# naver/dust3r

Measured on NVIDIA H100. Metric: image-pairs/sec (512x384, ViT-L/B+DPT), higher is better.
Workload: dtype bf16

## Files before the change

dust3r_b200/_lib.py:

```python
from __future__ import annotations

import ctypes as C
import os

from ._lib_fwd import Model

_HERE = os.path.dirname(os.path.abspath(__file__))
LIB_PATH = os.path.join(_HERE, 'libdust3r_b200.so')

_lib = None


class D3RError(RuntimeError):
    pass


class AlignDesc(C.Structure):
    _fields_ = [
        ('n_imgs', C.c_int32), ('n_edges', C.c_int32), ('n_entries', C.c_int32), ('n_chunks', C.c_int32),
        ('max_deg', C.c_int32), ('max_chunks', C.c_int32), ('chunk_px', C.c_int32), ('dist_l2', C.c_int32), ('norm_pw_scale', C.c_int32),
        ('tied_focal', C.c_int32), ('eval_only', C.c_int32),
        ('base_scale', C.c_float), ('pw_break', C.c_float), ('focal_break', C.c_float), ('adam_eps', C.c_float),
        ('beta1', C.c_float), ('beta2', C.c_float),
        ('img_hw', C.c_void_p), ('img_pix_off', C.c_void_p), ('img_ent_ptr', C.c_void_p),
# ... 52 lines not shown
    'd3r_align_stream_warps_per_cta': (i32, []),
    'd3r_align_stream_max_window': (i32, []),
    'd3r_align_pack_entries': (i32, [vp, i32, i32, i32, i32, vp, vp]),
    'd3r_gemm_bf16': (i32, [vp, vp, vp, vp, vp, vp, i32, i32, i32, i64, u32, vp, vp, i32, i32, i32, vp]),
    'd3r_conv3x3_bf16': (i32, [vp, vp, vp, vp, vp, vp, vp, i32, i32, i32, i32, i32, u32, vp]),
    'd3r_attention_hd64': (i32, [vp, i64, vp, i64, vp, i64, vp, i64, i32, i32, i32, i32, f32, vp]),
    'd3r_conv_transpose_bf16': (i32, [vp, vp, vp, vp, i32, i32, i32, i32, i32, i32, vp]),
    'd3r_conv3x3_head_tail': (i32, [vp, vp, vp, vp, vp, vp, vp, i32, i32, i32, i32, i32, f32, f32, vp]),
    'd3r_layernorm_bf16': (i32, [vp, vp, vp, vp, i32, i32, f32, vp]),
    'd3r_upsample2x_bf16': (i32, [vp, vp, i32, i32, i32, i32, i32, i32, vp]),
    'd3r_im2col_3x3_s2_bf16': (i32, [vp, vp, i32, i32, i32, i32, vp]),
    'd3r_patch_im2col16': (i32, [vp, vp, i32, i32, i32, vp]),
    'd3r_linear_head_postprocess': (i32, [vp, vp, vp, i32, i32, i32, i32, i32, i32, f32, f32, vp]),
    'd3r_set_gemm_impl': (None, [i32]),
    'd3r_set_gemm_store': (None, [i32]),
    'd3r_set_conv_store': (None, [i32]),
    'd3r_set_attention_impl': (None, [i32]),
    'd3r_clean_pointcloud': (i32, [i32, vp, vp, i32, vp, vp, vp, vp, vp, f32, f32, vp]),
    'd3r_procrustes_moments': (i32, [i32, i32, vp, vp, vp, vp, vp]),
    'd3r_weiszfeld_focal': (i32, [i32, i32, i32, vp, vp, i32, vp, vp]),
    'd3r_nearest_neighbours': (i32, [i32, i32, vp, vp, vp, vp]),
    'd3r_image_resize_crop_normalize': (i32, [vp, i32, i32, i32, i32, vp, vp, i32, vp, vp, i32, i32, i32, i32, i32, i32, i32,
                                              vp, vp, vp, vp]),
    'd3r_sizeof_jpeg_desc': (i32, []),
    'd3r_jpeg_decode_workspace_bytes': (i64, [_JPEG, i64]),
    'd3r_jpeg_decode': (i32, [_JPEG, vp, i64, vp, vp, vp, i64, vp]),
    'd3r_segment_sky_workspace_bytes': (i64, [i32, i64]),
    'd3r_segment_sky': (i32, [i32, vp, vp, i32, i64, vp, vp, vp, i64, vp]),
    'd3r_nanmedian_workspace_bytes': (i64, [i32]),
    'd3r_segmented_nanmedian': (i32, [i32, i64, vp, vp, vp, i64, vp]),
# ... 88 lines not shown
```

dust3r_b200/csrc/gemm_host.cu:

```cuda
#include "gemm_wgmma.cuh"
#include "gemm_host.h"
#include "prof.h"

namespace d3r {
namespace gemm {

static int pick_block_n(int N, int mode, uint32_t flags, int conv_m_tiles = 0) {
  if (flags & F_HEAD_FINAL) return 128;
  if (conv_m_tiles > 0) return (N == 256 && (conv_m_tiles + 1) / 2 >= 4 * (num_sms() / 2)) ? 256 : 128;
  if (N % 256 == 0 && pick_epi(mode, flags) != EPI_GENERIC) return 256;
  if (N % 128 == 0) return 128;
  if (N % 64 == 0) return 64;
  return (N > 128) ? 128 : 64;
}

static int g_impl = 2;
constexpr int kPairMinKb = 4;
static bool use_pair(int bn, int num_kb) { return bn >= 128 && (g_impl == 1 || (g_impl == 2 && num_kb >= kPairMinKb)); }

static int g_store = 1;
static int g_conv_store = 1;

static int grid_for(bool pair, int m_tiles, int n_tiles) {
  if (pair) {
    const int items = ((m_tiles + 1) / 2) * n_tiles;
    const int max_clusters = num_sms() / 2;
    return 2 * (items < max_clusters ? items : max_clusters);
  }
  const int items = m_tiles * n_tiles;
  return items < num_sms() ? items : num_sms();
}

static const char* prof_tag(const Params& p, int bn, bool pair) {
  return (p.mode == 1) ? ((p.flags & F_HEAD_FINAL) ? (pair ? "conv3x3_head_tail_2cta" : "conv3x3_head_tail")
                                                   : (pair ? "conv3x3_wgmma_2cta" : "conv3x3_wgmma"))
                       : (bn == 256 ? (pair ? "gemm_wgmma_2cta_bn256" : "gemm_wgmma_bn256")
                                    : (pair ? "gemm_wgmma_2cta_bn128" : (bn == 128 ? "gemm_wgmma_bn128" : "gemm_wgmma_bn64")));
}

template <int BN, int EPI, bool PAIR, bool TMA_STORE = false>
static int launch(const CUtensorMap& ta, const CUtensorMap& tb, const CUtensorMap& to, const Params& p, int m_tiles, int n_tiles,
                  cudaStream_t st) {
  constexpr int kSmem = Cfg<BN, TMA_STORE>::kSmemBytes;
  static unsigned long long attr_devices = 0;
  if (first_launch_on_this_device(attr_devices))
    D3R_CUDA(cudaFuncSetAttribute(gemm_kernel<BN, EPI, PAIR, TMA_STORE>, cudaFuncAttributeMaxDynamicSharedMemorySize, kSmem));
  const int grid = grid_for(PAIR, m_tiles, n_tiles);
  char detail[96];
  snprintf(detail, sizeof(detail), "M=%d N=%d K=%d flags=0x%x mode=%d epi=%d", p.M, p.N, p.K, (unsigned)p.flags, p.mode, EPI);
  prof::Scope scope(prof_tag(p, BN, PAIR), st, 2.0 * double(p.M) * double(p.N) * double(p.K), 0.0, 1, detail);
  D3R_CUDA(pdl::launch_clustered(gemm_kernel<BN, EPI, PAIR, TMA_STORE>, dim3(grid), dim3(kNumThreads), size_t(kSmem), st, PAIR ? 2 : 1,
                                 ta, tb, to, p));
  D3R_LAUNCH_CHECK();
  return D3R_OK;
}

template <int BN, bool PAIR>
static int launch_conv(const CUtensorMap& ta, const CUtensorMap& tb, const CUtensorMap& to, const ConvMaps& cm, const Params& p,
                       int m_tiles, int n_tiles, cudaStream_t st) {
  constexpr int kSmem = Cfg<BN, true>::kSmemBytes;
  static unsigned long long attr_devices = 0;
  if (first_launch_on_this_device(attr_devices))
    D3R_CUDA(cudaFuncSetAttribute(conv_kernel<BN, PAIR>, cudaFuncAttributeMaxDynamicSharedMemorySize, kSmem));
  const int grid = grid_for(PAIR, m_tiles, n_tiles);
  char detail[96];
  snprintf(detail, sizeof(detail), "M=%d N=%d K=%d flags=0x%x mode=%d epi=%d", p.M, p.N, p.K, (unsigned)p.flags, p.mode, EPI_GENERIC);
  prof::Scope scope(prof_tag(p, BN, PAIR), st, 2.0 * double(p.M) * double(p.N) * double(p.K), 0.0, 1, detail);
  D3R_CUDA(pdl::launch_clustered(conv_kernel<BN, PAIR>, dim3(grid), dim3(kNumThreads), size_t(kSmem), st, PAIR ? 2 : 1, ta, tb, to, cm, p));
  D3R_LAUNCH_CHECK();
  return D3R_OK;
}

template <int BN, bool PAIR>
static int dispatch_epi(int epi, const CUtensorMap& ta, const CUtensorMap& tb, const CUtensorMap* to, const Params& p, int m_tiles,
                        int n_tiles, cudaStream_t st) {
  if constexpr (BN == 256) {
    if (to) {
      switch (epi) {
        case EPI_RESID: return launch<BN, EPI_RESID, PAIR, true>(ta, tb, *to, p, m_tiles, n_tiles, st);
        case EPI_ACT: return launch<BN, EPI_ACT, PAIR, true>(ta, tb, *to, p, m_tiles, n_tiles, st);
        case EPI_ROPE: return launch<BN, EPI_ROPE, PAIR, true>(ta, tb, *to, p, m_tiles, n_tiles, st);
      }
    }
  }
  switch (epi) {
    case EPI_RESID: return launch<BN, EPI_RESID, PAIR>(ta, tb, tb, p, m_tiles, n_tiles, st);
    case EPI_ACT: return launch<BN, EPI_ACT, PAIR>(ta, tb, tb, p, m_tiles, n_tiles, st);
    case EPI_ROPE: return launch<BN, EPI_ROPE, PAIR>(ta, tb, tb, p, m_tiles, n_tiles, st);
  }
  if constexpr (BN == 128) return launch<128, EPI_GENERIC, PAIR>(ta, tb, tb, p, m_tiles, n_tiles, st);
  set_error("no BLOCK_N %d kernel for the generic epilogue", BN);
  return D3R_ERR_INVALID;
}

static int dispatch(int bn, const CUtensorMap& ta, const CUtensorMap& tb, const CUtensorMap* to, const Params& p, int m_tiles,
                    cudaStream_t st) {
  const int n_tiles = (p.N + bn - 1) / bn;
  const int epi = (bn >= 128) ? pick_epi(p.mode, p.flags) : EPI_GENERIC;
  const bool pair = use_pair(bn, p.num_kb);
  switch (bn) {
    case 256: return pair ? dispatch_epi<256, true>(epi, ta, tb, to, p, m_tiles, n_tiles, st) : dispatch_epi<256, false>(epi, ta, tb, to, p, m_tiles, n_tiles, st);
    case 128: return pair ? dispatch_epi<128, true>(epi, ta, tb, nullptr, p, m_tiles, n_tiles, st) : dispatch_epi<128, false>(epi, ta, tb, nullptr, p, m_tiles, n_tiles, st);
    case 64: return launch<64, EPI_GENERIC, false>(ta, tb, tb, p, m_tiles, n_tiles, st);
  }
  set_error("unsupported BLOCK_N %d", bn);
  return D3R_ERR_INVALID;
}

static int make_tmap_b(CUtensorMap* m, const void* B, int N, int taps, int Kc, int bn, int num_kb, const char* op) {
  cuuint64_t dims[3] = {(cuuint64_t)Kc, (cuuint64_t)taps, (cuuint64_t)N};
  cuuint64_t str[2] = {(cuuint64_t)Kc * 2, (cuuint64_t)taps * Kc * 2};
  cuuint32_t box[3] = {(cuuint32_t)BLOCK_K, 1, (cuuint32_t)(use_pair(bn, num_kb) ? bn / 2 : bn)};
  return encode_tensor_map(m, B, 3, dims, str, box, op);
}

int gemm_bf16(const void* A, long long lda, const void* B, Params p, cudaStream_t st) {
  D3R_CHECK_ARG(A && B, "gemm: null operand");
  D3R_CHECK_ARG(p.M > 0 && p.N > 0 && p.K > 0, "gemm: bad shape %d %d %d", p.M, p.N, p.K);
  D3R_CHECK_ARG(p.N % 32 == 0, "gemm: N=%d must be a multiple of 32", p.N);
  D3R_CHECK_ARG(p.K % 8 == 0 && lda % 8 == 0, "gemm: K=%d / lda=%lld must be multiples of 8 (16-byte TMA strides)", p.K, lda);
  D3R_CHECK_ARG((reinterpret_cast<uintptr_t>(A) & 15) == 0 && (reinterpret_cast<uintptr_t>(B) & 15) == 0, "gemm: operands must be 16-byte aligned");
  p.mode = 0;
  p.num_kb = (p.K + BLOCK_K - 1) / BLOCK_K;
  const int bn = pick_block_n(p.N, p.mode, p.flags);
  CUtensorMap ta, tb;
  {
    cuuint64_t dims[2] = {(cuuint64_t)p.K, (cuuint64_t)p.M};
    cuuint64_t str[1] = {(cuuint64_t)lda * 2};
    cuuint32_t box[2] = {(cuuint32_t)BLOCK_K, (cuuint32_t)BLOCK_M};
    int rc = encode_tensor_map(&ta, A, 2, dims, str, box, "gemm");
    if (rc) return rc;
  }
  int rc = make_tmap_b(&tb, B, p.N, 1, p.K, bn, p.num_kb, "gemm");
  if (rc) return rc;
  CUtensorMap to;
  const bool f32 = (p.flags & F_RESID_INPLACE) != 0;
  const long long row_bytes = p.ldo * (f32 ? 4 : 2);
  const bool staged = g_store == 1 && bn == 256 && pick_epi(p.mode, p.flags) != EPI_GENERIC && p.ldo >= p.N && row_bytes % 16 == 0 &&
                      (reinterpret_cast<uintptr_t>(p.out) & 15) == 0;
  if (staged) {
    cuuint64_t dims[2] = {(cuuint64_t)p.N, (cuuint64_t)p.M};
    cuuint64_t str[1] = {(cuuint64_t)row_bytes};
    cuuint32_t box[2] = {(cuuint32_t)(f32 ? 32 : 64), 64};
    rc = encode_tensor_map(&to, p.out, 2, dims, str, box, "gemm output", f32 ? CU_TENSOR_MAP_DATA_TYPE_FLOAT32 : CU_TENSOR_MAP_DATA_TYPE_BFLOAT16);
    if (rc) return rc;
  }
  return dispatch(bn, ta, tb, staged ? &to : nullptr, p, (p.M + BLOCK_M - 1) / BLOCK_M, st);
}

static int make_tmap_conv_io(CUtensorMap* m, const void* base, int B, int H, int W, int C, int tile_w, const char* op) {
  const int bw = tile_w < 64 ? tile_w : 64;
  cuuint64_t dims[4] = {(cuuint64_t)C, (cuuint64_t)W, (cuuint64_t)H, (cuuint64_t)B};
  cuuint64_t str[3] = {(cuuint64_t)C * 2, (cuuint64_t)W * C * 2, (cuuint64_t)H * W * C * 2};
  cuuint32_t box[4] = {64, (cuuint32_t)bw, (cuuint32_t)(64 / bw), 1};
  return encode_tensor_map(m, base, 4, dims, str, box, op);
}

static bool aligned16(const void* ptr) { return (reinterpret_cast<uintptr_t>(ptr) & 15) == 0; }

int conv3x3_bf16(const void* x_nhwc, const void* w_packed, int B, int H, int W, int Cin, int Cout, Params p, cudaStream_t st) {
  D3R_CHECK_ARG(x_nhwc && w_packed, "conv3x3: null operand");
  D3R_CHECK_ARG(Cin % 8 == 0 && Cout % 32 == 0, "conv3x3: Cin=%d must be a multiple of 8 and Cout=%d of 32", Cin, Cout);
// ... 12 lines not shown
  p.tiles_y = (H + p.tile_h - 1) / p.tile_h;
  p.ldo = Cout;
  const int m_tiles = B * p.tiles_x * p.tiles_y;
  const bool staged = g_conv_store == 1 && (Cout == 256 || Cout == 128) && (p.flags & ~EpiMask<EPI_CONV>::value) == 0 &&
                      aligned16(p.out) && (!(p.flags & F_OUT2_RELU) || aligned16(p.out2)) && (!(p.flags & F_ADD0) || aligned16(p.add0)) &&
                      (!(p.flags & F_ADD1) || aligned16(p.add1));
  const int bn = pick_block_n(p.N, p.mode, p.flags, staged ? m_tiles : 0);
  CUtensorMap ta, tb;
  {
    cuuint64_t dims[4] = {(cuuint64_t)Cin, (cuuint64_t)W, (cuuint64_t)H, (cuuint64_t)B};
    cuuint64_t str[3] = {(cuuint64_t)Cin * 2, (cuuint64_t)W * Cin * 2, (cuuint64_t)H * W * Cin * 2};
    cuuint32_t box[4] = {(cuuint32_t)BLOCK_K, (cuuint32_t)p.tile_w, (cuuint32_t)p.tile_h, 1};
    int rc = encode_tensor_map(&ta, x_nhwc, 4, dims, str, box, "conv3x3");
    if (rc) return rc;
  }
  int rc = make_tmap_b(&tb, w_packed, Cout, 9, Cin, bn, p.num_kb, "conv3x3");
  if (rc) return rc;
  if (!staged) return dispatch(bn, ta, tb, nullptr, p, m_tiles, st);
  CUtensorMap to;
  ConvMaps cm;
  rc = make_tmap_conv_io(&to, p.out, B, H, W, Cout, p.tile_w, "conv3x3 output");
  if (rc) return rc;
  cm.out2 = cm.add0 = cm.add1 = to;
  const struct { uint32_t flag; const void* base; CUtensorMap* map; const char* op; } io[3] = {
      {F_OUT2_RELU, p.out2, &cm.out2, "conv3x3 out2"}, {F_ADD0, p.add0, &cm.add0, "conv3x3 add0"}, {F_ADD1, p.add1, &cm.add1, "conv3x3 add1"}};
  for (const auto& t : io) {
    if (!(p.flags & t.flag)) continue;
    rc = make_tmap_conv_io(t.map, t.base, B, H, W, Cout, p.tile_w, t.op);
    if (rc) return rc;
  }
  const int n_tiles = Cout / bn;
  const bool pair = use_pair(bn, p.num_kb);
  if (bn == 256) return pair ? launch_conv<256, true>(ta, tb, to, cm, p, m_tiles, n_tiles, st) : launch_conv<256, false>(ta, tb, to, cm, p, m_tiles, n_tiles, st);
// ... 29 lines not shown
  p.w4 = w4; p.b4 = b4;
  p.pts3d = pts3d; p.conf = conf;
  p.depth_mode = depth_mode; p.conf_mode = conf_mode;
  p.conf_min = conf_min; p.conf_max = conf_max;
  return conv3x3_bf16(x_nhwc, w_packed, B, H, W, 128, 128, p, st);
}

}
}

using namespace d3r;

extern "C" void d3r_set_gemm_impl(int32_t impl) { gemm::g_impl = impl; }
extern "C" void d3r_set_gemm_store(int32_t store) { gemm::g_store = store; }
extern "C" void d3r_set_conv_store(int32_t store) { gemm::g_conv_store = store; }

extern "C" int d3r_gemm_bf16(const void* A, const void* B, void* out, const float* bias, const void* add0, void* out2,
                             int32_t M, int32_t N, int32_t K, int64_t ldo, uint32_t flags, const float* rope_cos,
                             const float* rope_sin, int32_t rope_cols, int32_t tokens_per_img, int32_t grid_w, void* stream) {
  gemm::Params p{};
  p.M = M; p.N = N; p.K = K;
  p.flags = flags;
  p.out = out; p.out2 = out2; p.add0 = add0; p.bias = bias; p.ldo = ldo;
  p.rope_cos = rope_cos; p.rope_sin = rope_sin; p.rope_cols = rope_cols; p.tokens_per_img = tokens_per_img; p.grid_w = grid_w;
  D3R_CHECK_ARG(!(flags & gemm::F_BIAS) || bias, "gemm: F_BIAS without bias");
  D3R_CHECK_ARG(!(flags & gemm::F_ROPE) || (rope_cos && rope_sin && tokens_per_img > 0 && grid_w > 0), "gemm: F_ROPE without tables");
  D3R_CHECK_ARG(!(flags & (gemm::F_CONVT | gemm::F_HEAD_FINAL)),
                "gemm: F_CONVT / F_HEAD_FINAL have their own entry points, d3r_conv_transpose_bf16 / d3r_conv3x3_head_tail");
  return gemm::gemm_bf16(A, K, B, p, (cudaStream_t)stream);
}
// ... 23 lines not shown
```

dust3r_b200/csrc/gemm_wgmma.cuh:

```cuda
#pragma once
#include "d3r_common.cuh"
#include "sm90_ptx.cuh"
#include "pdl.cuh"

namespace d3r {
namespace gemm {

constexpr int BLOCK_M = 128;
constexpr int BLOCK_K = 64;
constexpr int WGMMA_K = 16;
constexpr int kNumThreads = 384;
constexpr int kConsumerWarps = 8;

enum : uint32_t {
  F_BIAS = 1u << 0,
  F_GELU = 1u << 1,
  F_RELU = 1u << 2,
  F_OUT_F32 = 1u << 3,
  F_RESID_INPLACE = 1u << 4,
  F_ADD0 = 1u << 5,
  F_ADD1 = 1u << 6,
  F_OUT2_RELU = 1u << 7,
  F_ROPE = 1u << 8,
  F_CONVT = 1u << 9,
// ... 33 lines not shown
template <> struct EpiMask<EPI_ROPE> { static constexpr uint32_t value = F_BIAS | F_ROPE; };
template <> struct EpiMask<EPI_CONV> { static constexpr uint32_t value = F_BIAS | F_RELU | F_ADD0 | F_ADD1 | F_OUT2_RELU; };

struct ConvMaps {
  CUtensorMap out2, add0, add1;
};

__host__ __device__ inline int pick_epi(int mode, uint32_t flags) {
  if (mode != 0) return EPI_GENERIC;
  if ((flags & ~F_BIAS) == F_RESID_INPLACE) return EPI_RESID;
  if ((flags & ~EpiMask<EPI_ACT>::value) == 0) return EPI_ACT;
  if ((flags & ~EpiMask<EPI_ROPE>::value) == 0) return EPI_ROPE;
  return EPI_GENERIC;
}

template <int BLOCK_N, bool TMA_STORE = false>
struct Cfg {
  static constexpr int kStageA = BLOCK_M * BLOCK_K * 2;
  static constexpr int kStageB = BLOCK_N * BLOCK_K * 2;
  static constexpr int kStages = (BLOCK_N == 256) ? 4 : (BLOCK_N == 128) ? 6 : 8;
  static constexpr int kRing = kStages * (kStageA + kStageB);
  static constexpr int kOutBuf = 64 * 128;
  static constexpr int kStaging = TMA_STORE ? 2 * 2 * kOutBuf : 0;
  static constexpr int kSmemBytes = kRing + kStaging + 1024  + 256  + (TMA_STORE ? 0 : (4 * 128 + 16) * 4) ;
  static_assert(kSmemBytes <= 227 * 1024, "shared memory of one CTA");
};

__device__ __forceinline__ float gelu_erf(float x) {
  constexpr float kU = 0.84932180028801904f;
  constexpr float kP = 0.3275911f * 0.70710678118654752f / kU;
  const float u = fabsf(x) * kU;
  const float t = ptx::rcp_approx(fmaf(kP, u, 1.f));
  float poly = fmaf(0.5f * 1.061405429f, t, 0.5f * -1.453152027f);
  poly = fmaf(poly, t, 0.5f * 1.421413741f);
  poly = fmaf(poly, t, 0.5f * -0.284496736f);
  poly = fmaf(poly, t, 0.5f * 0.254829592f);
  const float e = ptx::ex2_approx(-u * u);
  const float h = x * (poly * t * e);
  return fmaxf(x, 0.f) - fabsf(h);
}

template <int BLOCK_N, int EPI, bool PAIR, bool TMA_STORE>
__device__ __forceinline__ void gemm_body(const CUtensorMap& tmap_a, const CUtensorMap& tmap_b, const CUtensorMap& tmap_o,
                                          const ConvMaps* cm, const Params& p) {
  static_assert(EPI == EPI_CONV ? (TMA_STORE && (BLOCK_N == 256 || BLOCK_N == 128))
                                : (!TMA_STORE || (BLOCK_N == 256 && EPI != EPI_GENERIC)),
                "TMA-store epilogue: specialised projection epilogues on 128x256 tiles, the conv epilogue on 128x256 / 128x128");
  using C = Cfg<BLOCK_N, TMA_STORE>;
  extern __shared__ uint8_t smem_raw[];
  uint8_t* smem = reinterpret_cast<uint8_t*>((reinterpret_cast<uintptr_t>(smem_raw) + 1023) & ~uintptr_t(1023));
  uint8_t* smem_a = smem;
  uint8_t* smem_b = smem + C::kStages * C::kStageA;
  uint8_t* smem_o = smem + C::kRing;
  uint64_t* bars = reinterpret_cast<uint64_t*>(smem + C::kRing + C::kStaging);
  uint64_t* full_bar = bars;
  uint64_t* empty_bar = bars + C::kStages;
  uint64_t* add_bar = bars + 2 * C::kStages;
  float* s_w4 = reinterpret_cast<float*>(reinterpret_cast<uint8_t*>(bars) + 256);

  const int warp = threadIdx.x >> 5, lane = threadIdx.x & 31;
  const uint32_t rank = PAIR ? ptx::cluster_ctarank() : 0u;
  const int n_tiles = (p.N + BLOCK_N - 1) / BLOCK_N;
  const int m_tiles = (p.mode == 1) ? p.cB * p.tiles_y * p.tiles_x : (p.M + BLOCK_M - 1) / BLOCK_M;
// ... 86 lines not shown
        } else {
          ptx::mbar_arrive(ptx::smem_u32(&empty_bar[s]));
        }
      }
    };
    const bool conv_issuer = EPI == EPI_CONV && (threadIdx.x & 127) == 0;
    const bool conv_two = EPI == EPI_CONV && (flags & (F_OUT2_RELU | F_ADD1)) != 0;
    const bool conv_add = EPI == EPI_CONV && (flags & (F_ADD0 | F_ADD1)) != 0;
    uint32_t add_phase = 0;
    auto conv_box = [&](int tm, int& bx, int& by, int& bb) {
      bb = tm / (p.tiles_y * p.tiles_x);
      const int r = tm - bb * (p.tiles_y * p.tiles_x);
      bx = (r % p.tiles_x) * p.tile_w + (64 * wg) % p.tile_w;
      by = (r / p.tiles_x) * p.tile_h + (64 * wg) / p.tile_w;
    };
    auto out_buf = [&](int i) { return ptx::smem_u32(smem_o + (wg * 2 + i) * C::kOutBuf); };
    auto issue_addends = [&](int tm, int ch) {
      int bx, by, bb;
      conv_box(tm, bx, by, bb);
      const uint32_t b0 = conv_two ? out_buf(0) : out_buf(out_chunk & 1);
      if (conv_two) ptx::bulk_wait_group_read<0>();
      else ptx::bulk_wait_group_read<1>();
      const uint32_t bar = ptx::smem_u32(&add_bar[wg]);
      ptx::mbar_arrive_expect_tx(bar, uint32_t(C::kOutBuf) * (((flags & F_ADD0) ? 1u : 0u) + ((flags & F_ADD1) ? 1u : 0u)));
      if (flags & F_ADD0) ptx::tma_load_4d(b0, &cm->add0, bar, ch, bx, by, bb);
      if (flags & F_ADD1) ptx::tma_load_4d(out_buf(1), &cm->add1, bar, ch, bx, by, bb);
    };
    for (int item = first_item; item < total_items; item += item_stride) {
      const int tn = item % n_tiles, tm = (item / n_tiles) * (PAIR ? 2 : 1) + int(rank);
      if constexpr (EPI == EPI_CONV) {
        if (conv_add && conv_issuer) issue_addends(tm, tn * BLOCK_N);
// ... 7 lines not shown
#pragma unroll
        for (int k = 0; k < BLOCK_K / WGMMA_K; ++k) {
          if constexpr (BLOCK_N == 256) ptx::wgmma_m64n256k16_ss(acc, da + uint64_t(2 * k), db + uint64_t(2 * k), (kb | k) != 0 ? 1u : 0u);
          else if constexpr (BLOCK_N == 128) ptx::wgmma_m64n128k16_ss(acc, da + uint64_t(2 * k), db + uint64_t(2 * k), (kb | k) != 0 ? 1u : 0u);
          else ptx::wgmma_m64n64k16_ss(acc, da + uint64_t(2 * k), db + uint64_t(2 * k), (kb | k) != 0 ? 1u : 0u);
        }
        ptx::wgmma_commit();
        ptx::wgmma_wait<1>();
        if (prev >= 0) release(prev);
        prev = stage;
        if (++stage == C::kStages) { stage = 0; phase ^= 1; }
      }
      ptx::wgmma_wait<0>();
      ptx::reg_fence(acc);
      release(prev);

      bool valid[2];
      long long row_off[2];
      int tok[2] = {0, 0};
      long long pix[2] = {0, 0};
      int ct_b[2] = {0, 0}, ct_iy[2] = {0, 0}, ct_ix[2] = {0, 0};
#pragma unroll
      for (int h = 0; h < 2; ++h) {
        const int row_in_tile = wg * 64 + wq * 16 + (lane >> 2) + 8 * h;
        if (p.mode == 1) {
          const int cb = tm / (p.tiles_y * p.tiles_x);
          const int r = tm - cb * (p.tiles_y * p.tiles_x);
          const int y = (r / p.tiles_x) * p.tile_h + row_in_tile / p.tile_w;
          const int x = (r % p.tiles_x) * p.tile_w + row_in_tile % p.tile_w;
          valid[h] = (tm < m_tiles) && (y < p.cH) && (x < p.cW);
// ... 99 lines not shown
            ptx::bulk_commit_group();
          }
          ++out_chunk;
          if (conv_add && conv_issuer && c + 1 < BLOCK_N / 64) issue_addends(tm, ch + 64);
        }
        continue;
      }
      if constexpr (TMA_STORE) {
        constexpr bool kF32 = (EPI == EPI_RESID);
        constexpr int kChunkCols = kF32 ? 32 : 64;
        constexpr int kChunkNB = kChunkCols / 8;
        const bool issuer = (threadIdx.x & 127) == 0;
        const uint32_t sw = lane >> 2;
#pragma unroll
        for (int c = 0; c < BLOCK_N / kChunkCols; ++c) {
          const uint32_t buf = ptx::smem_u32(smem_o + (wg * 2 + (out_chunk & 1)) * C::kOutBuf);
#pragma unroll
          for (int j = 0; j < kChunkNB; ++j)
#pragma unroll
            for (int h = 0; h < 2; ++h) {
              const uint32_t row = wq * 16 + (lane >> 2) + 8 * h;
              float v0 = acc[4 * (c * kChunkNB + j) + 2 * h], v1 = acc[4 * (c * kChunkNB + j) + 2 * h + 1];
              if (flags & F_RELU) { v0 = fmaxf(v0, 0.f); v1 = fmaxf(v1, 0.f); }
              if constexpr (kF32) {
                ptx::st_shared_v2_f32(buf + row * 128 + (((2 * j + (q >> 1)) ^ sw) << 4) + (q & 1) * 8, v0, v1);
              } else {
                ptx::st_shared_b32(buf + row * 128 + ((j ^ sw) << 4) + q * 4, pack_bf16x2(v0, v1));
              }
            }
          ptx::fence_proxy_async();
          if (issuer) ptx::bulk_wait_group_read<0>();
          ptx::named_bar_sync(1 + wg, 128);
          if (issuer) {
            const int c0 = tn * BLOCK_N + c * kChunkCols, r0 = tm * BLOCK_M + wg * 64;
            if constexpr (kF32) ptx::tma_reduce_add_2d(&tmap_o, buf, c0, r0);
            else ptx::tma_store_2d(&tmap_o, buf, c0, r0);
            ptx::bulk_commit_group();
          }
          ++out_chunk;
        }
        continue;
      }
      if (flags & F_HEAD_FINAL) {
        float head_acc[2][4] = {{0.f, 0.f, 0.f, 0.f}, {0.f, 0.f, 0.f, 0.f}};
#pragma unroll
        for (int j = 0; j < kNB; ++j)
// ... 58 lines not shown
          } else {
            *reinterpret_cast<uint32_t*>(reinterpret_cast<__nv_bfloat16*>(p.out) + off) = pack_bf16x2(v0, v1);
            if (flags & F_OUT2_RELU)
              *reinterpret_cast<uint32_t*>(reinterpret_cast<__nv_bfloat16*>(p.out2) + off) = pack_bf16x2(fmaxf(v0, 0.f), fmaxf(v1, 0.f));
          }
        }
      }
    }
    if constexpr (TMA_STORE) {
      if ((threadIdx.x & 127) == 0) ptx::bulk_wait_group<0>();
    }
  }
  if constexpr (PAIR) ptx::cluster_sync();
}

template <int BLOCK_N, int EPI, bool PAIR, bool TMA_STORE>
__global__ void __launch_bounds__(kNumThreads, 1)
gemm_kernel(const __grid_constant__ CUtensorMap tmap_a, const __grid_constant__ CUtensorMap tmap_b,
            const __grid_constant__ CUtensorMap tmap_o, const Params p) {
  gemm_body<BLOCK_N, EPI, PAIR, TMA_STORE>(tmap_a, tmap_b, tmap_o, nullptr, p);
}

template <int BLOCK_N, bool PAIR>
__global__ void __launch_bounds__(kNumThreads, 1)
conv_kernel(const __grid_constant__ CUtensorMap tmap_a, const __grid_constant__ CUtensorMap tmap_b,
            const __grid_constant__ CUtensorMap tmap_o, const __grid_constant__ ConvMaps cm, const Params p) {
  gemm_body<BLOCK_N, EPI_CONV, PAIR, true>(tmap_a, tmap_b, tmap_o, &cm, p);
}

}
}
```

dust3r_b200/csrc/sm90_ptx.cuh:

```cuda
#pragma once
#include <cuda.h>
#include <cuda_runtime.h>
#include <cuda_bf16.h>
#include <cstdint>

namespace d3r {
namespace ptx {

__device__ __forceinline__ uint32_t smem_u32(const void* p) { return static_cast<uint32_t>(__cvta_generic_to_shared(p)); }

__device__ __forceinline__ bool elect_one() {
  uint32_t pred = 0;
  asm volatile(
      "{\n"
      ".reg .b32 %%rx;\n"
      ".reg .pred %%px;\n"
      "elect.sync %%rx|%%px, %1;\n"
      "@%%px mov.s32 %0, 1;\n"
      "}\n"
      : "+r"(pred)
      : "r"(0xffffffffu));
  return pred != 0;
}

// ... 90 lines not shown
               ::"l"(reinterpret_cast<uint64_t>(tmap)), "r"(src), "r"(c0), "r"(c1) : "memory");
}
__device__ __forceinline__ void bulk_commit_group() { asm volatile("cp.async.bulk.commit_group;" ::: "memory"); }
template <int N> __device__ __forceinline__ void bulk_wait_group_read() { asm volatile("cp.async.bulk.wait_group.read %0;" ::"n"(N) : "memory"); }
template <int N> __device__ __forceinline__ void bulk_wait_group() { asm volatile("cp.async.bulk.wait_group %0;" ::"n"(N) : "memory"); }
__device__ __forceinline__ void st_shared_b32(uint32_t addr, uint32_t v) { asm volatile("st.shared.b32 [%0], %1;" ::"r"(addr), "r"(v) : "memory"); }
__device__ __forceinline__ uint32_t ld_shared_b32(uint32_t addr) {
  uint32_t v;
  asm volatile("ld.shared.b32 %0, [%1];" : "=r"(v) : "r"(addr) : "memory");
  return v;
}
__device__ __forceinline__ void st_shared_v2_f32(uint32_t addr, float a, float b) {
  asm volatile("st.shared.v2.f32 [%0], {%1, %2};" ::"r"(addr), "f"(a), "f"(b) : "memory");
}
__device__ __forceinline__ void named_bar_sync(uint32_t id, uint32_t count) { asm volatile("bar.sync %0, %1;" ::"r"(id), "r"(count) : "memory"); }

__device__ __forceinline__ uint32_t cluster_ctarank() {
  uint32_t r;
  asm volatile("mov.u32 %0, %%cluster_ctarank;" : "=r"(r));
  return r;
}
__device__ __forceinline__ void cluster_sync() {
  asm volatile("barrier.cluster.arrive.release.aligned;\nbarrier.cluster.wait.acquire.aligned;" ::: "memory");
}
__device__ __forceinline__ void mbar_arrive_cluster(uint32_t bar, uint32_t rank) {
  asm volatile(
      "{\n"
      ".reg .b32 raddr;\n"
      "mapa.shared::cluster.u32 raddr, %0, %1;\n"
      "mbarrier.arrive.shared::cluster.b64 _, [raddr];\n"
// ... 89 lines not shown
```

include/dust3r_b200.h:

```cpp
#ifndef DUST3R_B200_H_
#define DUST3R_B200_H_

#include <stddef.h>
#include <stdint.h>

#ifdef __cplusplus
extern "C" {
#endif

#define D3R_OK 0
#define D3R_ERR_INVALID (-1)
#define D3R_ERR_CUDA (-2)
#define D3R_ERR_UNSUPPORTED_DEVICE (-3)

const char* d3r_last_error(void);
int d3r_abi_version(void);
int d3r_check_device(void);

long long d3r_launch_count(void);
void d3r_launch_count_reset(void);
void d3r_prof_enable(int on);
int d3r_prof_report(char* buf, int cap);
int d3r_prof_dump(char* buf, int cap);

// ... 130 lines not shown
int d3r_layernorm_bf16(const float* x_dev, const float* g_dev, const float* b_dev, void* out_dev, int32_t M, int32_t C, float eps,
                       void* stream);

int d3r_upsample2x_bf16(const void* x_dev, void* out_dev, int32_t B, int32_t H, int32_t W, int32_t C, int32_t Ho, int32_t Wo,
                        void* stream);

int d3r_im2col_3x3_s2_bf16(const void* x_dev, void* out_dev, int32_t B, int32_t H, int32_t W, int32_t C, void* stream);

int d3r_patch_im2col16(const float* img_dev, void* out_dev, int32_t B, int32_t H, int32_t W, void* stream);

int d3r_linear_head_postprocess(const float* feat_dev, float* pts3d_dev, float* conf_dev, int32_t B, int32_t gh, int32_t gw,
                                int32_t nch, int32_t depth_mode, int32_t conf_mode, float conf_min, float conf_max, void* stream);

void d3r_set_gemm_impl(int32_t impl);
void d3r_set_gemm_store(int32_t store);
void d3r_set_conv_store(int32_t store);

void d3r_set_attention_impl(int32_t impl);

int d3r_clean_pointcloud(int32_t n_imgs, const int32_t* hw_dev, const int64_t* off_dev, int32_t max_area, const float* pts3d_dev,
                         float* conf_dev, const float* depth_dev, const float* K_dev, const float* cams_dev, float tol,
                         float bad_conf, void* stream);
int d3r_procrustes_moments(int32_t n_problems, int32_t n_points, const float* x_dev, const float* y_dev, const float* w_dev,
                           double* out_dev, void* stream);
int d3r_weiszfeld_focal(int32_t n_maps, int32_t H, int32_t W, const float* pts3d_dev, const float* pp_dev, int32_t steps,
                        float* focal_dev, void* stream);
int d3r_nearest_neighbours(int32_t n_queries, int32_t n_points, const float* queries_dev, const float* points_dev, int32_t* nn_dev,
                           void* stream);
int d3r_image_resize_crop_normalize(const uint8_t* src_dev, int32_t H0, int32_t W0, int32_t H1, int32_t W1,
                                    const int32_t* xbounds_dev, const int32_t* xcoefs_dev, int32_t kx,
// ... 121 lines not shown
```

Before: 231.4.

## Add ping-pong warpgroup schedule for 128x256 TMA-store projection GEMMs

Adds a ping-pong consumer schedule for the BN=256 TMA-store projection GEMMs. Each consumer warpgroup computes a full 128x128 half-tile while the other runs its epilogue, ordered by named barriers, with a 6-stage ring of half-width B tiles. A heuristic picks it for GELU GEMMs and for K<=768 GEMMs that do not accumulate in place; the rest take the cooperative kernel, which now uses four output staging buffers and three stages for ACT/ROPE. The aim is to hide epilogue cost behind MMA, at the price of more scheduling complexity and a shallower ring in the cooperative path.

```diff
diff --git a/dust3r_b200/_lib.py b/dust3r_b200/_lib.py
--- a/dust3r_b200/_lib.py
+++ b/dust3r_b200/_lib.py
@@ -90,6 +90,7 @@
     'd3r_linear_head_postprocess': (i32, [vp, vp, vp, i32, i32, i32, i32, i32, i32, f32, f32, vp]),
     'd3r_set_gemm_impl': (None, [i32]),
     'd3r_set_gemm_store': (None, [i32]),
+    'd3r_set_gemm_pingpong': (None, [i32]),
     'd3r_set_conv_store': (None, [i32]),
     'd3r_set_attention_impl': (None, [i32]),
     'd3r_clean_pointcloud': (i32, [i32, vp, vp, i32, vp, vp, vp, vp, vp, f32, f32, vp]),
diff --git a/dust3r_b200/csrc/gemm_host.cu b/dust3r_b200/csrc/gemm_host.cu
--- a/dust3r_b200/csrc/gemm_host.cu
+++ b/dust3r_b200/csrc/gemm_host.cu
@@ -21,6 +21,12 @@
 static int g_store = 1;
 static int g_conv_store = 1;
 
+static int g_pingpong = 2;
+static bool use_pingpong(const Params& p) {
+  if (g_pingpong != 2) return g_pingpong == 1;
+  return (p.flags & F_GELU) || (p.K <= 768 && !(p.flags & F_RESID_INPLACE));
+}
+
 static int grid_for(bool pair, int m_tiles, int n_tiles) {
   if (pair) {
     const int items = ((m_tiles + 1) / 2) * n_tiles;
@@ -38,19 +44,22 @@
                                     : (pair ? "gemm_wgmma_2cta_bn128" : (bn == 128 ? "gemm_wgmma_bn128" : "gemm_wgmma_bn64")));
 }
 
-template <int BN, int EPI, bool PAIR, bool TMA_STORE = false>
+template <int BN, int EPI, bool PAIR, bool TMA_STORE = false, bool COOP = false>
 static int launch(const CUtensorMap& ta, const CUtensorMap& tb, const CUtensorMap& to, const Params& p, int m_tiles, int n_tiles,
                   cudaStream_t st) {
   constexpr int kSmem = Cfg<BN, TMA_STORE>::kSmemBytes;
+  const auto kernel = [] {
+    if constexpr (COOP) return &gemm_coop_kernel<EPI, PAIR>;
+    else return &gemm_kernel<BN, EPI, PAIR, TMA_STORE>;
+  }();
   static unsigned long long attr_devices = 0;
   if (first_launch_on_this_device(attr_devices))
-    D3R_CUDA(cudaFuncSetAttribute(gemm_kernel<BN, EPI, PAIR, TMA_STORE>, cudaFuncAttributeMaxDynamicSharedMemorySize, kSmem));
+    D3R_CUDA(cudaFuncSetAttribute(kernel, cudaFuncAttributeMaxDynamicSharedMemorySize, kSmem));
   const int grid = grid_for(PAIR, m_tiles, n_tiles);
   char detail[96];
   snprintf(detail, sizeof(detail), "M=%d N=%d K=%d flags=0x%x mode=%d epi=%d", p.M, p.N, p.K, (unsigned)p.flags, p.mode, EPI);
   prof::Scope scope(prof_tag(p, BN, PAIR), st, 2.0 * double(p.M) * double(p.N) * double(p.K), 0.0, 1, detail);
-  D3R_CUDA(pdl::launch_clustered(gemm_kernel<BN, EPI, PAIR, TMA_STORE>, dim3(grid), dim3(kNumThreads), size_t(kSmem), st, PAIR ? 2 : 1,
-                                 ta, tb, to, p));
+  D3R_CUDA(pdl::launch_clustered(kernel, dim3(grid), dim3(kNumThreads), size_t(kSmem), st, PAIR ? 2 : 1, ta, tb, to, p));
   D3R_LAUNCH_CHECK();
   return D3R_OK;
 }
@@ -72,15 +81,21 @@
 }
 
 template <int BN, bool PAIR>
-static int dispatch_epi(int epi, const CUtensorMap& ta, const CUtensorMap& tb, const CUtensorMap* to, const Params& p, int m_tiles,
-                        int n_tiles, cudaStream_t st) {
+static int dispatch_epi(int epi, const CUtensorMap& ta, const CUtensorMap& tb, const CUtensorMap* to, bool pingpong, const Params& p,
+                        int m_tiles, int n_tiles, cudaStream_t st) {
   if constexpr (BN == 256) {
-    if (to) {
+    if (to && pingpong) {
       switch (epi) {
         case EPI_RESID: return launch<BN, EPI_RESID, PAIR, true>(ta, tb, *to, p, m_tiles, n_tiles, st);
         case EPI_ACT: return launch<BN, EPI_ACT, PAIR, true>(ta, tb, *to, p, m_tiles, n_tiles, st);
         case EPI_ROPE: return launch<BN, EPI_ROPE, PAIR, true>(ta, tb, *to, p, m_tiles, n_tiles, st);
       }
+    } else if (to) {
+      switch (epi) {
+        case EPI_RESID: return launch<BN, EPI_RESID, PAIR, true, true>(ta, tb, *to, p, m_tiles, n_tiles, st);
+        case EPI_ACT: return launch<BN, EPI_ACT, PAIR, true, true>(ta, tb, *to, p, m_tiles, n_tiles, st);
+        case EPI_ROPE: return launch<BN, EPI_ROPE, PAIR, true, true>(ta, tb, *to, p, m_tiles, n_tiles, st);
+      }
     }
   }
   switch (epi) {
@@ -93,24 +108,29 @@
   return D3R_ERR_INVALID;
 }
 
-static int dispatch(int bn, const CUtensorMap& ta, const CUtensorMap& tb, const CUtensorMap* to, const Params& p, int m_tiles,
-                    cudaStream_t st) {
+static int dispatch(int bn, const CUtensorMap& ta, const CUtensorMap& tb, const CUtensorMap* to, bool pingpong, const Params& p,
+                    int m_tiles, cudaStream_t st) {
   const int n_tiles = (p.N + bn - 1) / bn;
   const int epi = (bn >= 128) ? pick_epi(p.mode, p.flags) : EPI_GENERIC;
   const bool pair = use_pair(bn, p.num_kb);
   switch (bn) {
-    case 256: return pair ? dispatch_epi<256, true>(epi, ta, tb, to, p, m_tiles, n_tiles, st) : dispatch_epi<256, false>(epi, ta, tb, to, p, m_tiles, n_tiles, st);
-    case 128: return pair ? dispatch_epi<128, true>(epi, ta, tb, nullptr, p, m_tiles, n_tiles, st) : dispatch_epi<128, false>(epi, ta, tb, nullptr, p, m_tiles, n_tiles, st);
+    case 256:
+      return pair ? dispatch_epi<256, true>(epi, ta, tb, to, pingpong, p, m_tiles, n_tiles, st)
+                  : dispatch_epi<256, false>(epi, ta, tb, to, pingpong, p, m_tiles, n_tiles, st);
+    case 128:
+      return pair ? dispatch_epi<128, true>(epi, ta, tb, nullptr, false, p, m_tiles, n_tiles, st)
+                  : dispatch_epi<128, false>(epi, ta, tb, nullptr, false, p, m_tiles, n_tiles, st);
     case 64: return launch<64, EPI_GENERIC, false>(ta, tb, tb, p, m_tiles, n_tiles, st);
   }
   set_error("unsupported BLOCK_N %d", bn);
   return D3R_ERR_INVALID;
 }
 
-static int make_tmap_b(CUtensorMap* m, const void* B, int N, int taps, int Kc, int bn, int num_kb, const char* op) {
+static int make_tmap_b(CUtensorMap* m, const void* B, int N, int taps, int Kc, int bn, int num_kb, bool pingpong, const char* op) {
   cuuint64_t dims[3] = {(cuuint64_t)Kc, (cuuint64_t)taps, (cuuint64_t)N};
   cuuint64_t str[2] = {(cuuint64_t)Kc * 2, (cuuint64_t)taps * Kc * 2};
-  cuuint32_t box[3] = {(cuuint32_t)BLOCK_K, 1, (cuuint32_t)(use_pair(bn, num_kb) ? bn / 2 : bn)};
+  const int rows = (use_pair(bn, num_kb) ? bn / 2 : bn) / (pingpong ? 2 : 1);
+  cuuint32_t box[3] = {(cuuint32_t)BLOCK_K, 1, (cuuint32_t)rows};
   return encode_tensor_map(m, B, 3, dims, str, box, op);
 }
 
@@ -131,13 +151,14 @@
     int rc = encode_tensor_map(&ta, A, 2, dims, str, box, "gemm");
     if (rc) return rc;
   }
-  int rc = make_tmap_b(&tb, B, p.N, 1, p.K, bn, p.num_kb, "gemm");
-  if (rc) return rc;
   CUtensorMap to;
   const bool f32 = (p.flags & F_RESID_INPLACE) != 0;
   const long long row_bytes = p.ldo * (f32 ? 4 : 2);
   const bool staged = g_store == 1 && bn == 256 && pick_epi(p.mode, p.flags) != EPI_GENERIC && p.ldo >= p.N && row_bytes % 16 == 0 &&
                       (reinterpret_cast<uintptr_t>(p.out) & 15) == 0;
+  const bool pingpong = staged && use_pingpong(p);
+  int rc = make_tmap_b(&tb, B, p.N, 1, p.K, bn, p.num_kb, pingpong, "gemm");
+  if (rc) return rc;
   if (staged) {
     cuuint64_t dims[2] = {(cuuint64_t)p.N, (cuuint64_t)p.M};
     cuuint64_t str[1] = {(cuuint64_t)row_bytes};
@@ -145,7 +166,7 @@
     rc = encode_tensor_map(&to, p.out, 2, dims, str, box, "gemm output", f32 ? CU_TENSOR_MAP_DATA_TYPE_FLOAT32 : CU_TENSOR_MAP_DATA_TYPE_BFLOAT16);
     if (rc) return rc;
   }
-  return dispatch(bn, ta, tb, staged ? &to : nullptr, p, (p.M + BLOCK_M - 1) / BLOCK_M, st);
+  return dispatch(bn, ta, tb, staged ? &to : nullptr, pingpong, p, (p.M + BLOCK_M - 1) / BLOCK_M, st);
 }
 
 static int make_tmap_conv_io(CUtensorMap* m, const void* base, int B, int H, int W, int C, int tile_w, const char* op) {
@@ -188,9 +209,9 @@
     int rc = encode_tensor_map(&ta, x_nhwc, 4, dims, str, box, "conv3x3");
     if (rc) return rc;
   }
-  int rc = make_tmap_b(&tb, w_packed, Cout, 9, Cin, bn, p.num_kb, "conv3x3");
+  int rc = make_tmap_b(&tb, w_packed, Cout, 9, Cin, bn, p.num_kb, false, "conv3x3");
   if (rc) return rc;
-  if (!staged) return dispatch(bn, ta, tb, nullptr, p, m_tiles, st);
+  if (!staged) return dispatch(bn, ta, tb, nullptr, false, p, m_tiles, st);
   CUtensorMap to;
   ConvMaps cm;
   rc = make_tmap_conv_io(&to, p.out, B, H, W, Cout, p.tile_w, "conv3x3 output");
@@ -250,6 +271,7 @@
 extern "C" void d3r_set_gemm_impl(int32_t impl) { gemm::g_impl = impl; }
 extern "C" void d3r_set_gemm_store(int32_t store) { gemm::g_store = store; }
 extern "C" void d3r_set_conv_store(int32_t store) { gemm::g_conv_store = store; }
+extern "C" void d3r_set_gemm_pingpong(int32_t pingpong) { gemm::g_pingpong = pingpong; }
 
 extern "C" int d3r_gemm_bf16(const void* A, const void* B, void* out, const float* bias, const void* add0, void* out2,
                              int32_t M, int32_t N, int32_t K, int64_t ldo, uint32_t flags, const float* rope_cos,
diff --git a/dust3r_b200/csrc/gemm_wgmma.cuh b/dust3r_b200/csrc/gemm_wgmma.cuh
--- a/dust3r_b200/csrc/gemm_wgmma.cuh
+++ b/dust3r_b200/csrc/gemm_wgmma.cuh
@@ -71,17 +71,21 @@
   return EPI_GENERIC;
 }
 
-template <int BLOCK_N, bool TMA_STORE = false>
+template <int BLOCK_N, bool TMA_STORE = false, int OUT_BUFS = 2>
 struct Cfg {
   static constexpr int kStageA = BLOCK_M * BLOCK_K * 2;
   static constexpr int kStageB = BLOCK_N * BLOCK_K * 2;
-  static constexpr int kStages = (BLOCK_N == 256) ? 4 : (BLOCK_N == 128) ? 6 : 8;
+  static constexpr int kStages = (BLOCK_N == 256) ? (OUT_BUFS == 4 ? 3 : 4) : (BLOCK_N == 128) ? 6 : 8;
   static constexpr int kRing = kStages * (kStageA + kStageB);
   static constexpr int kOutBuf = 64 * 128;
-  static constexpr int kStaging = TMA_STORE ? 2 * 2 * kOutBuf : 0;
+  static constexpr int kOutBufs = OUT_BUFS;
+  static constexpr int kStaging = TMA_STORE ? 2 * OUT_BUFS * kOutBuf : 0;
   static constexpr int kSmemBytes = kRing + kStaging + 1024  + 256  + (TMA_STORE ? 0 : (4 * 128 + 16) * 4) ;
   static_assert(kSmemBytes <= 227 * 1024, "shared memory of one CTA");
 };
+
+template <int BLOCK_N, int EPI, bool TMA_STORE>
+constexpr int kOutBufsOf = (BLOCK_N == 256 && TMA_STORE && (EPI == EPI_ACT || EPI == EPI_ROPE)) ? 4 : 2;
 
 __device__ __forceinline__ float gelu_erf(float x) {
   constexpr float kU = 0.84932180028801904f;
@@ -103,7 +107,7 @@
   static_assert(EPI == EPI_CONV ? (TMA_STORE && (BLOCK_N == 256 || BLOCK_N == 128))
                                 : (!TMA_STORE || (BLOCK_N == 256 && EPI != EPI_GENERIC)),
                 "TMA-store epilogue: specialised projection epilogues on 128x256 tiles, the conv epilogue on 128x256 / 128x128");
-  using C = Cfg<BLOCK_N, TMA_STORE>;
+  using C = Cfg<BLOCK_N, TMA_STORE, kOutBufsOf<BLOCK_N, EPI, TMA_STORE>>;
   extern __shared__ uint8_t smem_raw[];
   uint8_t* smem = reinterpret_cast<uint8_t*>((reinterpret_cast<uintptr_t>(smem_raw) + 1023) & ~uintptr_t(1023));
   uint8_t* smem_a = smem;
@@ -220,7 +224,7 @@
       bx = (r % p.tiles_x) * p.tile_w + (64 * wg) % p.tile_w;
       by = (r / p.tiles_x) * p.tile_h + (64 * wg) / p.tile_w;
     };
-    auto out_buf = [&](int i) { return ptx::smem_u32(smem_o + (wg * 2 + i) * C::kOutBuf); };
+    auto out_buf = [&](int i) { return ptx::smem_u32(smem_o + (wg * C::kOutBufs + i) * C::kOutBuf); };
     auto issue_addends = [&](int tm, int ch) {
       int bx, by, bb;
       conv_box(tm, bx, by, bb);
@@ -258,6 +262,9 @@
       ptx::wgmma_wait<0>();
       ptx::reg_fence(acc);
       release(prev);
+#ifdef D3R_GEMM_EPILOGUE_OFF
+      if constexpr (TMA_STORE && EPI != EPI_CONV) continue;
+#endif
 
       bool valid[2];
       long long row_off[2];
@@ -387,7 +394,7 @@
         const uint32_t sw = lane >> 2;
 #pragma unroll
         for (int c = 0; c < BLOCK_N / kChunkCols; ++c) {
-          const uint32_t buf = ptx::smem_u32(smem_o + (wg * 2 + (out_chunk & 1)) * C::kOutBuf);
+          const uint32_t buf = out_buf(out_chunk % C::kOutBufs);
 #pragma unroll
           for (int j = 0; j < kChunkNB; ++j)
 #pragma unroll
@@ -402,7 +409,7 @@
               }
             }
           ptx::fence_proxy_async();
-          if (issuer) ptx::bulk_wait_group_read<0>();
+          if (issuer) ptx::bulk_wait_group_read<C::kOutBufs - 2>();
           ptx::named_bar_sync(1 + wg, 128);
           if (issuer) {
             const int c0 = tn * BLOCK_N + c * kChunkCols, r0 = tm * BLOCK_M + wg * 64;
@@ -491,11 +498,241 @@
   if constexpr (PAIR) ptx::cluster_sync();
 }
 
+template <int EPI, bool PAIR>
+__device__ __forceinline__ void gemm_body_pingpong(const CUtensorMap& tmap_a, const CUtensorMap& tmap_b, const CUtensorMap& tmap_o,
+                                                   const Params& p) {
+  static_assert(EPI == EPI_RESID || EPI == EPI_ACT || EPI == EPI_ROPE, "ping-pong consumers: the projections' epilogues");
+  constexpr int kHalfN = 128;
+  static_assert(kHalfN % 64 == 0, "a warpgroup's columns are whole RoPE heads");
+  constexpr int kStageA = BLOCK_M * BLOCK_K * 2;
+  constexpr int kStageB = kHalfN * BLOCK_K * 2;
+  constexpr int kStages = 6;
+  using C = Cfg<256, true>;
+  static_assert(kStages * (kStageA + kStageB) == C::kRing, "the ping-pong ring takes the place of gemm_body's");
+  static_assert(2 * kStages * 8 <= 256, "barriers");
+  constexpr uint32_t kMathBar = 3;
+  extern __shared__ uint8_t smem_raw[];
+  uint8_t* smem = reinterpret_cast<uint8_t*>((reinterpret_cast<uintptr_t>(smem_raw) + 1023) & ~uintptr_t(1023));
+  uint8_t* smem_a = smem;
+  uint8_t* smem_b = smem + kStages * kStageA;
+  uint8_t* smem_o = smem + C::kRing;
+  uint64_t* bars = reinterpret_cast<uint64_t*>(smem + C::kRing + C::kStaging);
+  uint64_t* full_bar = bars;
+  uint64_t* empty_bar = bars + kStages;
+
+  const int warp = threadIdx.x >> 5, lane = threadIdx.x & 31;
+  const uint32_t rank = PAIR ? ptx::cluster_ctarank() : 0u;
+  const int num_kb = p.num_kb;
+  const int n_tiles = p.N / 256;
+  const int m_tiles = (p.M + BLOCK_M - 1) / BLOCK_M;
+  const int m_groups = PAIR ? (m_tiles + 1) / 2 : m_tiles;
+  const int total_items = m_groups * n_tiles;
+  const int first_item = PAIR ? blockIdx.x / 2 : blockIdx.x;
+  const int item_stride = PAIR ? gridDim.x / 2 : gridDim.x;
+
+  if (threadIdx.x == 0) {
+    ptx::prefetch_tmap(&tmap_a);
+    ptx::prefetch_tmap(&tmap_b);
+    ptx::prefetch_tmap(&tmap_o);
+    for (int s = 0; s < kStages; ++s) {
+      ptx::mbar_init(ptx::smem_u32(&full_bar[s]), 1);
+      ptx::mbar_init(ptx::smem_u32(&empty_bar[s]), (PAIR ? 2 : 1) * 4);
+    }
+    ptx::fence_barrier_init();
+  }
+  __syncthreads();
+  if constexpr (PAIR) ptx::cluster_sync();
+  pdl::sync_with_predecessor();
+
+  if (warp < 4) {
+    ptx::setmaxnreg_dec<40>();
+    if (warp == 0 && ptx::elect_one()) {
+      int stage = 0;
+      uint32_t phase = 0;
+      for (int item = first_item; item < total_items; item += item_stride) {
+        const int tn = item % n_tiles, tm = (item / n_tiles) * (PAIR ? 2 : 1) + int(rank);
+        for (int half = 0; half < 2; ++half) {
+          for (int kb = 0; kb < num_kb; ++kb) {
+            ptx::mbar_wait(ptx::smem_u32(&empty_bar[stage]), phase ^ 1);
+            const uint32_t fb = ptx::smem_u32(&full_bar[stage]);
+            ptx::mbar_arrive_expect_tx(fb, kStageA + kStageB);
+            const uint32_t sa = ptx::smem_u32(smem_a + stage * kStageA);
+            const uint32_t sb = ptx::smem_u32(smem_b + stage * kStageB);
+            ptx::tma_load_2d(sa, &tmap_a, fb, kb * BLOCK_K, tm * BLOCK_M);
+            const int n0 = tn * 256 + half * kHalfN;
+            if constexpr (PAIR) {
+              ptx::tma_load_3d_mc(sb + rank * (64 * BLOCK_K * 2), &tmap_b, fb, kb * BLOCK_K, 0, n0 + int(rank) * 64, 0x3);
+            } else {
+              ptx::tma_load_3d(sb, &tmap_b, fb, kb * BLOCK_K, 0, n0);
+            }
+            if (++stage == kStages) { stage = 0; phase ^= 1; }
+          }
+        }
+      }
+    }
+  } else {
+    ptx::setmaxnreg_inc<232>();
+    const int wg = (threadIdx.x >> 7) - 1;
+    const int wq = warp & 3;
+    const int q = lane & 3;
+    const uint32_t flags = p.flags & EpiMask<EPI>::value;
+    float acc[2][64];
+    int stage = 0;
+    uint32_t phase = 0;
+    auto advance = [&](int n) {
+      stage += n;
+      while (stage >= kStages) { stage -= kStages; phase ^= 1; }
+    };
+    if (wg == 1) advance(num_kb);
+    uint32_t out_chunk = 0;
+    auto release = [&](int s) {
+      if (lane == 0) {
+        if constexpr (PAIR) {
+          ptx::mbar_arrive_cluster(ptx::smem_u32(&empty_bar[s]), 0);
+          ptx::mbar_arrive_cluster(ptx::smem_u32(&empty_bar[s]), 1);
+        } else {
+          ptx::mbar_arrive(ptx::smem_u32(&empty_bar[s]));
+        }
+      }
+    };
+    for (int item = first_item; item < total_items; item += item_stride) {
+      const int tn = item % n_tiles, tm = (item / n_tiles) * (PAIR ? 2 : 1) + int(rank);
+      const bool last_item = item + item_stride >= total_items;
+      if (wg == 1 || item != first_item) ptx::named_bar_sync(kMathBar + wg, 256);
+      int prev = -1;
+      for (int kb = 0; kb < num_kb; ++kb) {
+        ptx::mbar_wait(ptx::smem_u32(&full_bar[stage]), phase);
+        const uint64_t da0 = ptx::desc_kmajor_sw128(ptx::smem_u32(smem_a + stage * kStageA));
+        const uint64_t da1 = ptx::desc_kmajor_sw128(ptx::smem_u32(smem_a + stage * kStageA + 64 * 128));
+        const uint64_t db = ptx::desc_kmajor_sw128(ptx::smem_u32(smem_b + stage * kStageB));
+        ptx::wgmma_fence();
+#pragma unroll
+        for (int k = 0; k < BLOCK_K / WGMMA_K; ++k) {
+          ptx::wgmma_m64n128k16_ss(acc[0], da0 + uint64_t(2 * k), db + uint64_t(2 * k), (kb | k) != 0 ? 1u : 0u);
+          ptx::wgmma_m64n128k16_ss(acc[1], da1 + uint64_t(2 * k), db + uint64_t(2 * k), (kb | k) != 0 ? 1u : 0u);
+        }
+        ptx::wgmma_commit();
+        ptx::wgmma_wait<1>();
+        if (prev >= 0) release(prev);
+        prev = stage;
+        advance(1);
+      }
+      if (wg == 0 || !last_item) ptx::named_bar_arrive(kMathBar + (wg ^ 1), 256);
+      ptx::wgmma_wait<0>();
+      ptx::reg_fence(acc[0]);
+      ptx::reg_fence(acc[1]);
+      release(prev);
+      advance(num_kb);
+#ifdef D3R_GEMM_EPILOGUE_OFF
+      continue;
+#endif
+
+      int tok[2][2] = {{0, 0}, {0, 0}};
+      if (flags & F_ROPE) {
+#pragma unroll
+        for (int mh = 0; mh < 2; ++mh)
+#pragma unroll
+          for (int h = 0; h < 2; ++h) tok[mh][h] = (tm * BLOCK_M + 64 * mh + wq * 16 + (lane >> 2) + 8 * h) % p.tokens_per_img;
+      }
+      if (flags & (F_BIAS | F_GELU)) {
+#pragma unroll
+        for (int j = 0; j < kHalfN / 8; ++j) {
+          const int c = tn * 256 + wg * kHalfN + 8 * j + 2 * q;
+          float2 b = make_float2(0.f, 0.f);
+          if (flags & F_BIAS) b = __ldg(reinterpret_cast<const float2*>(p.bias + c));
+#pragma unroll
+          for (int mh = 0; mh < 2; ++mh)
+#pragma unroll
+            for (int h = 0; h < 2; ++h) {
+              float& v0 = acc[mh][4 * j + 2 * h];
+              float& v1 = acc[mh][4 * j + 2 * h + 1];
+              v0 += b.x;
+              v1 += b.y;
+              if (flags & F_GELU) { v0 = gelu_erf(v0); v1 = gelu_erf(v1); }
+            }
+        }
+      }
+      if (flags & F_ROPE) {
+#pragma unroll
+        for (int cb = 0; cb < kHalfN / 32; ++cb) {
+          const int col0 = tn * 256 + wg * kHalfN + cb * 32;
+          if (col0 >= p.rope_cols) continue;
+#pragma unroll
+          for (int mh = 0; mh < 2; ++mh)
+#pragma unroll
+            for (int h = 0; h < 2; ++h) {
+              const int pos = ((col0 & 63) < 32) ? (tok[mh][h] / p.grid_w) : (tok[mh][h] % p.grid_w);
+#pragma unroll
+              for (int jj = 0; jj < 2; ++jj) {
+                const int k = 8 * jj + 2 * q;
+                const float2 cs = __ldg(reinterpret_cast<const float2*>(p.rope_cos + pos * 16 + k));
+                const float2 sn = __ldg(reinterpret_cast<const float2*>(p.rope_sin + pos * 16 + k));
+                const float cc[2] = {cs.x, cs.y}, ss[2] = {sn.x, sn.y};
+#pragma unroll
+                for (int e = 0; e < 2; ++e) {
+                  float& u = acc[mh][(4 * cb + jj) * 4 + 2 * h + e];
+                  float& w = acc[mh][(4 * cb + jj + 2) * 4 + 2 * h + e];
+                  const float u0 = u, w0 = w;
+                  u = u0 * cc[e] - w0 * ss[e];
+                  w = w0 * cc[e] + u0 * ss[e];
+                }
+              }
+            }
+        }
+      }
+      constexpr bool kF32 = (EPI == EPI_RESID);
+      constexpr int kChunkCols = kF32 ? 32 : 64;
+      constexpr int kChunkNB = kChunkCols / 8;
+      const bool issuer = (threadIdx.x & 127) == 0;
+      const uint32_t sw = lane >> 2;
+#pragma unroll
+      for (int mh = 0; mh < 2; ++mh)
+#pragma unroll
+        for (int c = 0; c < kHalfN / kChunkCols; ++c) {
+          const uint32_t buf = ptx::smem_u32(smem_o + (wg * 2 + (out_chunk & 1)) * C::kOutBuf);
+#pragma unroll
+          for (int j = 0; j < kChunkNB; ++j)
+#pragma unroll
+            for (int h = 0; h < 2; ++h) {
+              const uint32_t row = wq * 16 + (lane >> 2) + 8 * h;
+              float v0 = acc[mh][4 * (c * kChunkNB + j) + 2 * h], v1 = acc[mh][4 * (c * kChunkNB + j) + 2 * h + 1];
+              if (flags & F_RELU) { v0 = fmaxf(v0, 0.f); v1 = fmaxf(v1, 0.f); }
+              if constexpr (kF32) {
+                ptx::st_shared_v2_f32(buf + row * 128 + (((2 * j + (q >> 1)) ^ sw) << 4) + (q & 1) * 8, v0, v1);
+              } else {
+                ptx::st_shared_b32(buf + row * 128 + ((j ^ sw) << 4) + q * 4, pack_bf16x2(v0, v1));
+              }
+            }
+          ptx::fence_proxy_async();
+          if (issuer) ptx::bulk_wait_group_read<0>();
+          ptx::named_bar_sync(1 + wg, 128);
+          if (issuer) {
+            const int c0 = tn * 256 + wg * kHalfN + c * kChunkCols, r0 = tm * BLOCK_M + 64 * mh;
+            if constexpr (kF32) ptx::tma_reduce_add_2d(&tmap_o, buf, c0, r0);
+            else ptx::tma_store_2d(&tmap_o, buf, c0, r0);
+            ptx::bulk_commit_group();
+          }
+          ++out_chunk;
+        }
+    }
+    if ((threadIdx.x & 127) == 0) ptx::bulk_wait_group<0>();
+  }
+  if constexpr (PAIR) ptx::cluster_sync();
+}
+
 template <int BLOCK_N, int EPI, bool PAIR, bool TMA_STORE>
 __global__ void __launch_bounds__(kNumThreads, 1)
 gemm_kernel(const __grid_constant__ CUtensorMap tmap_a, const __grid_constant__ CUtensorMap tmap_b,
             const __grid_constant__ CUtensorMap tmap_o, const Params p) {
-  gemm_body<BLOCK_N, EPI, PAIR, TMA_STORE>(tmap_a, tmap_b, tmap_o, nullptr, p);
+  if constexpr (BLOCK_N == 256 && TMA_STORE) gemm_body_pingpong<EPI, PAIR>(tmap_a, tmap_b, tmap_o, p);
+  else gemm_body<BLOCK_N, EPI, PAIR, TMA_STORE>(tmap_a, tmap_b, tmap_o, nullptr, p);
+}
+
+template <int EPI, bool PAIR>
+__global__ void __launch_bounds__(kNumThreads, 1)
+gemm_coop_kernel(const __grid_constant__ CUtensorMap tmap_a, const __grid_constant__ CUtensorMap tmap_b,
+                 const __grid_constant__ CUtensorMap tmap_o, const Params p) {
+  gemm_body<256, EPI, PAIR, true>(tmap_a, tmap_b, tmap_o, nullptr, p);
 }
 
 template <int BLOCK_N, bool PAIR>
diff --git a/dust3r_b200/csrc/sm90_ptx.cuh b/dust3r_b200/csrc/sm90_ptx.cuh
--- a/dust3r_b200/csrc/sm90_ptx.cuh
+++ b/dust3r_b200/csrc/sm90_ptx.cuh
@@ -128,6 +128,7 @@
   asm volatile("st.shared.v2.f32 [%0], {%1, %2};" ::"r"(addr), "f"(a), "f"(b) : "memory");
 }
 __device__ __forceinline__ void named_bar_sync(uint32_t id, uint32_t count) { asm volatile("bar.sync %0, %1;" ::"r"(id), "r"(count) : "memory"); }
+__device__ __forceinline__ void named_bar_arrive(uint32_t id, uint32_t count) { asm volatile("bar.arrive %0, %1;" ::"r"(id), "r"(count) : "memory"); }
 
 __device__ __forceinline__ uint32_t cluster_ctarank() {
   uint32_t r;
diff --git a/include/dust3r_b200.h b/include/dust3r_b200.h
--- a/include/dust3r_b200.h
+++ b/include/dust3r_b200.h
@@ -168,6 +168,7 @@
 
 void d3r_set_gemm_impl(int32_t impl);
 void d3r_set_gemm_store(int32_t store);
+void d3r_set_gemm_pingpong(int32_t pingpong);
 void d3r_set_conv_store(int32_t store);
 
 void d3r_set_attention_impl(int32_t impl);
```

New measurement: 232.7, median of 6. About the same (+0.5%).
